# lukemelas/deep-spectral-segmentation

Hardware: AMD Instinct MI355X
Metric: images/sec end-to-end (features+eigs) at 480², K=5; eigvec cos-err vs CPU (higher is better)
Workload: dtype f16

## Files before the change

deep-spectral-segmentation_amd/build.py:

```python
from __future__ import annotations

import concurrent.futures as cf
import hashlib
import os
import shutil
import subprocess
import sys
from pathlib import Path

PKG = Path(__file__).resolve().parent
CSRC = PKG / "csrc"
LIBDIR = PKG / "lib"
LIB = LIBDIR / "libdss_hip.so"
SOURCES = ["lib.hip", "preprocess.hip", "layernorm.hip", "attention.hip", "linear384.hip", "affinity.hip", "eigs.hip", "segment.hip", "gemm.hip"]
ARCH = "gfx950"
FLAGS = ["--offload-arch=" + ARCH, "-O3", "-std=c++17", "-fPIC", "-Wall", "-Wno-unused-function"]
EXTRA_FLAGS = {"attention.hip": ["-fno-honor-nans", "-mno-amdgpu-ieee"]}


def _hipcc() -> str:
    for cand in (os.environ.get("HIPCC"), shutil.which("hipcc"), "/opt/rocm/bin/hipcc"):
        if cand and Path(cand).exists():
            return cand
    raise RuntimeError("hipcc not found (set HIPCC or install ROCm)")


def _digest() -> str:
    h = hashlib.sha256()
    for f in sorted(list(CSRC.glob("*.hip")) + list(CSRC.glob("*.h")) + [PKG.parent / "include" / "dss_hip.h"]):
        h.update(f.name.encode())
        h.update(f.read_bytes())
    h.update((" ".join(FLAGS) + repr(sorted(EXTRA_FLAGS.items()))).encode())
    return h.hexdigest()


def build(force: bool = False, verbose: bool = True) -> Path:
    LIBDIR.mkdir(exist_ok=True)
    stamp = LIBDIR / "libdss_hip.sha256"
    digest = _digest()
    if not force and LIB.exists() and stamp.exists() and stamp.read_text().strip() == digest:
        if verbose:
            print(f"[build] {LIB} is up to date")
        return LIB
    hipcc = _hipcc()
    objdir = LIBDIR / "obj"
    objdir.mkdir(exist_ok=True)

    def compile_one(src: str) -> Path:
        obj = objdir / (Path(src).stem + ".o")
        cmd = [hipcc, *FLAGS, *EXTRA_FLAGS.get(src, []), "-c", str(CSRC / src), "-o", str(obj)]
        r = subprocess.run(cmd, capture_output=True, text=True)
        if r.returncode != 0:
            raise RuntimeError(f"hipcc failed for {src}:\n{r.stdout}\n{r.stderr}")
        if verbose and r.stderr.strip():
            print(r.stderr, file=sys.stderr)
        return obj

    with cf.ThreadPoolExecutor(max_workers=min(8, len(SOURCES))) as ex:
        objs = list(ex.map(compile_one, SOURCES))
    rocm_lib = str(Path(hipcc).resolve().parent.parent / "lib")
    cmd = [hipcc, "--offload-arch=" + ARCH, "-shared", "-fPIC", "-o", str(LIB), *map(str, objs), "-L" + rocm_lib, "-lhipblaslt",
           "-Wl,-rpath," + rocm_lib]
    r = subprocess.run(cmd, capture_output=True, text=True)
    if r.returncode != 0:
        raise RuntimeError(f"link failed:\n{r.stdout}\n{r.stderr}")
    stamp.write_text(digest + "\n")
    if verbose:
        print(f"[build] wrote {LIB} ({LIB.stat().st_size} bytes)")
    return LIB


if __name__ == "__main__":
    build(force="--force" in sys.argv)
```

deep-spectral-segmentation_amd/hip.py:

```python
from __future__ import annotations

import ctypes
import functools
import os
from ctypes import c_char_p, c_float, c_int, c_size_t, c_uint, c_void_p
from pathlib import Path
from typing import Optional

import torch

PKG = Path(__file__).resolve().parent
LIB_PATH = PKG / "lib" / "libdss_hip.so"

DSS_F32, DSS_F16, DSS_BF16 = 0, 1, 2
_DTYPE_CODE = {torch.float32: DSS_F32, torch.float16: DSS_F16, torch.bfloat16: DSS_BF16}

SYMBOLS = {
    "dss_abi_version": (c_int, []),
    "dss_last_error": (c_char_p, []),
    "dss_target_arch": (c_char_p, []),
    "dss_preprocess_chw": (c_int, [c_void_p, c_void_p, c_int, c_int, c_int, c_void_p]),
    "dss_preprocess_patchify": (c_int, [c_void_p, c_void_p, c_int, c_int, c_int, c_int, c_int, c_void_p]),
    "dss_layernorm_fwd": (c_int, [c_void_p, c_void_p, c_int, c_int, c_void_p, c_void_p, c_void_p, c_int, c_int, c_int,
                                  c_float, c_void_p]),
    "dss_attention_fwd": (c_int, [c_void_p, c_int, c_void_p, c_int, c_int, c_int, c_float, c_int, c_void_p]),
    "dss_linear_k384": (c_int, [c_void_p, c_void_p, c_void_p, c_void_p, c_int, c_int, c_int, c_int, c_int, c_void_p]),
    "dss_linear_k768": (c_int, [c_void_p, c_void_p, c_void_p, c_void_p, c_int, c_int, c_int, c_int, c_int, c_void_p]),
    "dss_linear_lt_workspace_bytes": (c_size_t, []),
    "dss_linear_lt": (c_int, [c_void_p, c_void_p, c_void_p, c_void_p, ctypes.c_long, c_int, c_int, c_int, c_int, c_void_p, c_size_t,
                              c_void_p]),
    "dss_linear_lt_accumulate": (c_int, [c_void_p, c_void_p, c_void_p, c_void_p, ctypes.c_long, c_int, c_int, c_int, c_void_p, c_size_t,
                                         c_void_p]),
    "dss_linear_lt_describe": (c_int, [ctypes.c_long, c_int, c_int, c_int, c_int, c_int, c_size_t, c_char_p, c_size_t]),
    "dss_lnlinear_prepare": (c_int, [c_void_p, c_void_p, c_void_p, c_void_p, c_void_p, c_void_p, c_int, c_int, c_int,
                                     c_void_p]),
    "dss_lnlinear_k384": (c_int, [c_void_p, c_void_p, c_int, c_float, c_void_p, c_void_p, c_void_p, c_int, c_int, c_int,
                                  c_int, c_int, c_void_p]),
    "dss_lnlinear_k768": (c_int, [c_void_p, c_void_p, c_int, c_float, c_void_p, c_void_p, c_void_p, c_int, c_int, c_int,
                                  c_int, c_int, c_void_p]),
    "dss_lnlinear_kfeatures_k384": (c_int, [c_void_p, c_void_p, c_int, c_float, c_void_p, c_void_p, c_void_p, c_void_p,
                                            c_void_p, c_int, c_int, c_float, c_void_p]),
    "dss_lnlinear_kfeatures": (c_int, [c_void_p, c_void_p, c_int, c_float, c_void_p, c_void_p, c_void_p, c_void_p,
                                       c_void_p, c_int, c_int, c_int, c_float, c_int, c_void_p]),
    "dss_patch_embed_p16": (c_int, [c_void_p, c_void_p, c_void_p, c_void_p, c_void_p, c_int, c_int, c_int, c_int, c_int, c_void_p]),
    "dss_normalize_rows": (c_int, [c_void_p, c_void_p, c_int, c_int, c_float, c_void_p]),
    "dss_affinity_ld": (c_int, [c_int]),
    "dss_affinity_elems": (c_size_t, [c_int]),
    "dss_affinity": (c_int, [c_void_p, c_void_p, c_int, c_int, c_int, c_int, c_void_p]),
    "dss_affinity_split_workspace_bytes": (c_size_t, [c_int, c_int, c_int]),
    "dss_affinity_split": (c_int, [c_void_p, c_void_p, c_int, c_int, c_int, c_int, c_float, c_int, c_void_p, c_size_t,
                                   c_void_p]),
    "dss_affinity_split_u16": (c_int, [c_void_p, c_void_p, c_int, c_int, c_int, c_float, c_void_p, c_size_t, c_void_p]),
    "dss_affinity_fused_u16": (c_int, [c_void_p, c_void_p, c_int, c_int, c_int, c_float, c_void_p]),
    "dss_affinity_f16_u16": (c_int, [c_void_p, c_void_p, c_void_p, c_int, c_int, c_int, c_void_p]),
    "dss_kfeatures_finalize": (c_int, [c_void_p, c_void_p, c_void_p, c_void_p, c_void_p, c_int, c_int, c_int, c_float,
                                       c_void_p]),
    "dss_eigs_workspace_bytes": (c_size_t, [c_int, c_int, c_int, c_int]),
    "dss_laplacian_eigs_u16": (c_int, [c_void_p, c_int, c_int, c_int, c_void_p, c_void_p, c_void_p, c_int, c_float,
                                       c_int, c_void_p, c_size_t, c_void_p]),
    "dss_laplacian_eigs": (c_int, [c_void_p, c_int, c_int, c_int, c_void_p, c_void_p, c_void_p, c_int, c_float,
                                   c_int, c_void_p, c_size_t, c_void_p]),
    "dss_symmetric_eigs": (c_int, [c_void_p, c_int, c_int, c_int, c_int, c_void_p, c_void_p, c_void_p, c_int, c_float,
                                   c_int, c_void_p, c_size_t, c_void_p]),
    "dss_sign_rule": (c_int, [c_void_p, c_int, c_int, c_void_p]),
    "dss_fiedler_mask": (c_int, [c_void_p, c_void_p, c_int, c_int, c_int, c_int, c_float, c_void_p]),
    "dss_kmeans_segments": (c_int, [c_void_p, c_int, c_int, c_int, c_int, c_int, c_int, c_void_p, c_uint, c_int, c_float,
                                    c_int, c_int, c_int, c_void_p, c_void_p, c_void_p, c_void_p]),
}


class HipLibraryError(RuntimeError):
    """libdss_hip.so is missing, failed to load, or one of its entry points returned an error."""


_lib: Optional[ctypes.CDLL] = None

TIMERS: Optional[dict] = None
TIMER_SAMPLE = 1
TIMER_ALWAYS = ("laplacian_eigs", "affinity", "kfeatures_finalize", "lnlinear_kfeatures", "layernorm")


class _timed:

    def __init__(self, name: str, **meta):
        self.name, self.meta = name, meta

    def __enter__(self):
        self.on = False
        if TIMERS is not None:
            counts = TIMERS.setdefault("_launches", {})
            n = counts.get(self.name, 0)
            counts[self.name] = n + 1
            self.on = TIMER_SAMPLE <= 1 or self.name in TIMER_ALWAYS or n % TIMER_SAMPLE == 0
        if self.on:
            self.start = torch.cuda.Event(enable_timing=True)
            self.end = torch.cuda.Event(enable_timing=True)
            self.start.record()
        return self

    def __exit__(self, *exc):
        if self.on:
            self.end.record()
            TIMERS.setdefault(self.name, []).append((self.start, self.end, self.meta))
        return False


def load_library(path: Optional[Path] = None) -> ctypes.CDLL:
    global _lib
    if _lib is not None and path is None:
        return _lib
# ... 47 lines not shown
def preprocess_chw(img_u8: torch.Tensor) -> torch.Tensor:
    b, h, w, c = img_u8.shape
    assert c == 3 and img_u8.dtype == torch.uint8
    out = torch.empty((b, 3, h, w), dtype=torch.float32, device=img_u8.device)
    _check(load_library().dss_preprocess_chw(_dev(img_u8, "img"), _dev(out, "out"), b, h, w, _stream()),
           "dss_preprocess_chw")
    return out


def preprocess_patchify(img_u8: torch.Tensor, patch: int, dtype: torch.dtype) -> torch.Tensor:
    b, h, w, c = img_u8.shape
    assert c == 3 and img_u8.dtype == torch.uint8
    out = torch.empty((b, (h // patch) * (w // patch), 3 * patch * patch), dtype=dtype, device=img_u8.device)
    _check(load_library().dss_preprocess_patchify(_dev(img_u8, "img"), _dev(out, "out"), b, h, w, patch,
                                                  dtype_code(dtype), _stream()), "dss_preprocess_patchify")
    return out


ROW_MAJOR, PLANAR64 = 0, 1


def planar_to_rows(t: torch.Tensor) -> torch.Tensor:
    return t.permute(1, 0, 2).reshape(t.shape[1], t.shape[0] * 64)


def layernorm(x: torch.Tensor, gamma: torch.Tensor, beta: torch.Tensor, eps: float, out_dtype: torch.dtype,
              residual: Optional[torch.Tensor] = None, out: Optional[torch.Tensor] = None,
              residual_planar: bool = False) -> torch.Tensor:
    assert x.dtype == torch.float32
    d = x.shape[-1]
    rows = x.numel() // d
    if out is None:
        out = torch.empty(x.shape, dtype=out_dtype, device=x.device)
    rp, rc = (0, 0) if residual is None else (_dev(residual, "residual"), dtype_code(residual.dtype))
    if residual is not None:
        assert residual.shape == ((d // 64, rows, 64) if residual_planar else x.shape)
    layout = PLANAR64 if (residual is not None and residual_planar) else ROW_MAJOR
    with _timed("layernorm", rows=rows, d=d, res=residual is not None, out_bytes=out.element_size()):
        _check(load_library().dss_layernorm_fwd(_dev(x, "x"), rp, rc, layout, _dev(gamma, "gamma"), _dev(beta, "beta"),
                                                _dev(out, "out"), dtype_code(out.dtype), rows, d, float(eps),
                                                _stream()), "dss_layernorm_fwd")
    return out


def attention(qkv: torch.Tensor, heads: int, scale: float, out: Optional[torch.Tensor] = None,
              planar_bt: Optional[tuple] = None) -> torch.Tensor:
    if planar_bt is None:
        b, t, c3 = qkv.shape
        assert c3 == 3 * heads * 64, "head dim must be 64"
    else:
        b, t = planar_bt
        assert tuple(qkv.shape) == (3 * heads, b * t, 64), "planar qkv must be [3*heads, B*T, 64]"
    if out is None:
        out = torch.empty((b, t, heads * 64), dtype=qkv.dtype, device=qkv.device)
    with _timed("attention", b=b, t=t, heads=heads):
        _check(load_library().dss_attention_fwd(_dev(qkv, "qkv"), ROW_MAJOR if planar_bt is None else PLANAR64,
                                                _dev(out, "out"), b, t, heads, float(scale),
                                                dtype_code(qkv.dtype), _stream()),
               "dss_attention_fwd")
    return out


LINEAR_KRES_WIDTHS = {384: ("dss_linear_k384", 512), 768: ("dss_linear_k768", 256)}


def linear_kres(x: torch.Tensor, weight: torch.Tensor, bias: torch.Tensor, gelu: bool = False,
                planar: bool = False) -> torch.Tensor:
    k = x.shape[-1]
    if k not in LINEAR_KRES_WIDTHS:
        raise ValueError(f"linear_kres: reduction dimension must be one of {sorted(LINEAR_KRES_WIDTHS)} (got {k})")
    assert weight.shape[1] == k and x.dtype == weight.dtype == bias.dtype
    entry = LINEAR_KRES_WIDTHS[k][0]
    n = weight.shape[0]
    m = x.numel() // k
    shape = (n // 64, m, 64) if planar else (*x.shape[:-1], n)
    out = torch.empty(shape, dtype=x.dtype, device=x.device)
    with _timed("linear_kres", m=m, n=n, k=k, gelu=gelu):
        _check(getattr(load_library(), entry)(_dev(x, "x"), _dev(weight, "weight"), _dev(bias, "bias"), _dev(out, "out"),
                                              m, n, int(gelu), PLANAR64 if planar else ROW_MAJOR, dtype_code(x.dtype),
                                              _stream()), entry)
    return out


_LT_WORKSPACE: dict = {}


def _lt_workspace(device: torch.device) -> torch.Tensor:
    idx = device.index if device.index is not None else torch.cuda.current_device()
    if idx not in _LT_WORKSPACE:
        _LT_WORKSPACE[idx] = torch.empty(max(16, int(load_library().dss_linear_lt_workspace_bytes())), dtype=torch.uint8, device=device)
    return _LT_WORKSPACE[idx]


def linear_lt(x: torch.Tensor, weight: torch.Tensor, bias: Optional[torch.Tensor] = None, out_dtype: Optional[torch.dtype] = None,
              what: str = "") -> torch.Tensor:
    k = x.shape[-1]
    n = weight.shape[0]
    assert weight.shape[1] == k and x.dtype == weight.dtype and x.dtype in (torch.float16, torch.bfloat16)
    assert bias is None or (bias.dtype == x.dtype and tuple(bias.shape) == (n,))
    out_dtype = x.dtype if out_dtype is None else out_dtype
    m = x.numel() // k
    out = torch.empty((*x.shape[:-1], n), dtype=out_dtype, device=x.device)
    ws = _lt_workspace(x.device)
    with _timed("library_gemm", m=m, n=n, k=k, what=what):
        _check(load_library().dss_linear_lt(_dev(x, "x"), _dev(weight, "weight"), 0 if bias is None else _dev(bias, "bias"),
                                            _dev(out, "out"), m, n, k, dtype_code(x.dtype), dtype_code(out_dtype), ws.data_ptr(),
                                            ws.numel(), _stream()), "dss_linear_lt")
    return out


def linear_lt_accumulate(x: torch.Tensor, weight: torch.Tensor, bias: Optional[torch.Tensor], stream_x: torch.Tensor, what: str = "") -> torch.Tensor:
    k = x.shape[-1]
    n = weight.shape[0]
    assert weight.shape[1] == k and x.dtype == weight.dtype and x.dtype in (torch.float16, torch.bfloat16)
    assert bias is None or (bias.dtype == torch.float32 and tuple(bias.shape) == (n,))
    m = x.numel() // k
    assert stream_x.dtype == torch.float32 and stream_x.numel() == m * n
    ws = _lt_workspace(x.device)
    with _timed("library_gemm", m=m, n=n, k=k, what=what):
        _check(load_library().dss_linear_lt_accumulate(_dev(x, "x"), _dev(weight, "weight"), 0 if bias is None else _dev(bias, "bias"),
                                                       _dev(stream_x, "stream_x"), m, n, k, dtype_code(x.dtype), ws.data_ptr(), ws.numel(),
                                                       _stream()), "dss_linear_lt_accumulate")
    return stream_x


def linear_lt_describe(m: int, n: int, k: int, dtype: torch.dtype = torch.float16, out_dtype: Optional[torch.dtype] = None,
                       bias: bool = True) -> str:
    buf = ctypes.create_string_buffer(1 << 16)
    lib = load_library()
    _check(lib.dss_linear_lt_describe(m, n, k, dtype_code(dtype), dtype_code(out_dtype or dtype), int(bias),
                                      int(lib.dss_linear_lt_workspace_bytes()), buf, len(buf)), "dss_linear_lt_describe")
    return buf.value.decode(errors="replace")


IMAGENET_MEAN, IMAGENET_STD = (0.485, 0.456, 0.406), (0.229, 0.224, 0.225)


def patch_embed16_prepare(weight: torch.Tensor, bias: torch.Tensor, dtype: torch.dtype):
    d = weight.shape[0]
    w = weight.detach().double().reshape(d, 3, 16, 16)
    mean = torch.tensor(IMAGENET_MEAN, dtype=torch.float64, device=w.device).view(1, 3, 1, 1)
    std = torch.tensor(IMAGENET_STD, dtype=torch.float64, device=w.device).view(1, 3, 1, 1)
    bp = bias.detach().double() - (w * ((mean - 128.0 / 255.0) / std)).sum(dim=(1, 2, 3))
    wp = (w / (255.0 * std)).permute(0, 2, 3, 1).reshape(d, 768)
    return wp.to(dtype).contiguous(), bp.float().contiguous()


_ZERO_BIAS: dict = {}


def patch_embed16(img_u8: torch.Tensor, wp: torch.Tensor, bp: Optional[torch.Tensor], pos: torch.Tensor, x: torch.Tensor) -> torch.Tensor:
    assert img_u8.dtype == torch.uint8 and img_u8.dim() == 4 and img_u8.shape[-1] == 3 and img_u8.is_contiguous()
    b, h, w, _ = img_u8.shape
    n_p = (h // 16) * (w // 16)
    d = wp.shape[0]
    if bp is None:
        key = (d, wp.dtype, wp.device)
        if key not in _ZERO_BIAS:
            _ZERO_BIAS[key] = torch.zeros(d, dtype=wp.dtype, device=wp.device)
        bp = _ZERO_BIAS[key]
    else:
        bp = bp.to(wp.dtype)
    assert tuple(wp.shape) == (d, 768) and tuple(bp.shape) == (d,) and bp.dtype == wp.dtype
    assert pos.dtype == torch.float32 and tuple(pos.shape) == (n_p, d) and pos.is_contiguous()
    assert x.dtype == torch.float32 and tuple(x.shape) == (b, n_p + 1, d) and x.is_contiguous()
    with _timed("patch_embed", m=b * n_p, n=d, k=768):
# ... 275 lines not shown
```

deep-spectral-segmentation_amd/vit.py:

```python
from __future__ import annotations

import math
from pathlib import Path
from typing import Dict, Optional, Tuple

import torch
import torch.nn.functional as F

from . import hip
from .synthetic import VIT_CONFIGS

LN_EPS = 1e-6
_TUNING_FILE = Path(__file__).resolve().parent / "tuning" / "tunableop_gfx950.csv"
_gemm_tuning_ready = False


def setup_gemm_tuning(tune_new_shapes: bool = False, use_table: bool = True) -> None:
    global _gemm_tuning_ready
    if not use_table:
        return
    tun = torch.cuda.tunable
    if not _gemm_tuning_ready:
        tun.enable(True)
        if hasattr(tun, "write_file_on_exit"):
            tun.write_file_on_exit(False)
        tun.set_max_tuning_duration(15)
        if _TUNING_FILE.is_file():
            try:
                tun.read_file(str(_TUNING_FILE))
            except Exception as e:
                print(f"[dss] ignoring GEMM tuning table {_TUNING_FILE.name}: {e}")
        _gemm_tuning_ready = True
    tun.tuning_enable(bool(tune_new_shapes))


def interpolate_pos_encoding(pos_embed: torch.Tensor, patch: int, h: int, w: int) -> torch.Tensor:
    pos_embed = pos_embed.detach().float().cpu()
    n0 = pos_embed.shape[1] - 1
    hp, wp = h // patch, w // patch
    if hp * wp == n0 and h == w:
        return pos_embed.clone()
    dim = pos_embed.shape[-1]
    side = int(math.sqrt(n0))
    grid = pos_embed[:, 1:].reshape(1, side, side, dim).permute(0, 3, 1, 2)
    grid = F.interpolate(grid, scale_factor=((hp + 0.1) / side, (wp + 0.1) / side), mode="bicubic")
    if (grid.shape[-2], grid.shape[-1]) != (hp, wp):
        raise RuntimeError(f"pos-embed interpolation produced {tuple(grid.shape[-2:])}, wanted {(hp, wp)}")
    grid = grid.permute(0, 2, 3, 1).reshape(1, -1, dim)
    return torch.cat((pos_embed[:, :1], grid), dim=1)


class DinoViT:

    def __init__(self, model_name: str, state_dict: Dict[str, torch.Tensor], device: torch.device,
                 dtype: torch.dtype = torch.float16, k_proj_fp32: bool = False, gelu: str = "auto",
                 linear_kres: int = 2, fuse_ln: bool = True, gemm_tuning: str = "table", fuse_k: bool = True, fuse_pe: bool = True,
                 fuse_qkv768: bool = True, library_gemm: str = "lt", fc2_into_stream: bool = False):
        name = model_name.lower()
        if name not in VIT_CONFIGS:
            raise ValueError(f"Cannot get model: {model_name}")
        if dtype not in (torch.float16, torch.bfloat16):
            raise ValueError("compute dtype must be torch.float16 or torch.bfloat16")
        self.model_name = name
        self.embed_dim, self.depth, self.num_heads, self.patch_size = VIT_CONFIGS[name]
        self.device, self.dtype = torch.device(device), dtype
        self.k_proj_fp32 = k_proj_fp32
        if gelu not in ("auto", "erf", "erf_f16", "tanh_fused"):
            raise ValueError("gelu must be 'auto', 'erf' (DINO's exact GELU, fp32 arithmetic), 'erf_f16' (the same function evaluated on "
                             "packed f16: f16 operands and the K-resident fc1 kernel only) or 'tanh_fused'")
        if gelu == "auto":
            gelu = "erf_f16" if self.embed_dim == 384 else "erf"
        if gelu == "erf_f16" and (dtype != torch.float16 or linear_kres < 2 or self.embed_dim not in hip.LINEAR_KRES_WIDTHS):
            gelu = "erf"
        self.gelu = gelu
        self._gelu_code = 2 if gelu == "erf_f16" else 1
        if linear_kres not in (0, 1, 2):
            raise ValueError("linear_kres must be 0, 1 or 2")
        self.linear_k384 = int(linear_kres)
        self.fuse_ln = bool(fuse_ln)
        self.fuse_k = bool(fuse_k)
        self.fuse_qkv768 = bool(fuse_qkv768)
        if library_gemm not in ("lt", "torch"):
            raise ValueError("library_gemm must be 'lt' (dss_linear_lt) or 'torch' (F.linear)")
        self.library_gemm = library_gemm
        self.fc2_into_stream = bool(fc2_into_stream) and library_gemm == "lt"
        d = self.embed_dim
        sd = state_dict
        need = ["cls_token", "pos_embed", "patch_embed.proj.weight", "patch_embed.proj.bias"]
        for i in range(self.depth):
            for s in ("norm1.weight", "norm1.bias", "attn.qkv.weight", "attn.qkv.bias", "attn.proj.weight",
                      "attn.proj.bias", "norm2.weight", "norm2.bias", "mlp.fc1.weight", "mlp.fc1.bias",
                      "mlp.fc2.weight", "mlp.fc2.bias"):
                need.append(f"blocks.{i}.{s}")
        missing = [k for k in need if k not in sd]
        if missing:
            raise KeyError(f"state_dict is missing {len(missing)} DINO ViT keys, e.g. {missing[:3]}")

        def lp(t):
            return t.detach().to(self.device, dtype).contiguous()

        def f32(t):
            return t.detach().to(self.device, torch.float32).contiguous()

        self.cls_token = sd["cls_token"].detach().float().cpu()
        self.pos_embed = sd["pos_embed"].detach().float().cpu()
        self.pe_w = lp(sd["patch_embed.proj.weight"].reshape(d, -1))
        self.pe_b = lp(sd["patch_embed.proj.bias"])
        self.pe16 = None
        if self.patch_size == 16 and fuse_pe and fuse_ln and linear_kres and d % 64 == 0:
            self.pe16 = hip.patch_embed16_prepare(sd["patch_embed.proj.weight"].to(self.device), sd["patch_embed.proj.bias"].to(self.device), dtype)
        self.blocks = []
        for i in range(self.depth):
            p = f"blocks.{i}."
            self.blocks.append(dict(
                n1w=f32(sd[p + "norm1.weight"]), n1b=f32(sd[p + "norm1.bias"]),
                qkv_w=lp(sd[p + "attn.qkv.weight"]), qkv_b=lp(sd[p + "attn.qkv.bias"]),
                k_w32=f32(sd[p + "attn.qkv.weight"][d:2 * d]), k_b32=f32(sd[p + "attn.qkv.bias"][d:2 * d]),
                k_w=lp(sd[p + "attn.qkv.weight"][d:2 * d]),
                proj_w=lp(sd[p + "attn.proj.weight"]), proj_b=lp(sd[p + "attn.proj.bias"]),
                n2w=f32(sd[p + "norm2.weight"]), n2b=f32(sd[p + "norm2.bias"]),
                fc1_w=lp(sd[p + "mlp.fc1.weight"]), fc1_b=lp(sd[p + "mlp.fc1.bias"]),
                fc2_w=lp(sd[p + "mlp.fc2.weight"]), fc2_b=lp(sd[p + "mlp.fc2.bias"]), fc2_b32=f32(sd[p + "mlp.fc2.bias"]),
            ))
        hip.load_library()
        if self.fuse_ln and self.linear_k384 and d in hip.LINEAR_KRES_WIDTHS:
            for i, blk in enumerate(self.blocks):
                p = f"blocks.{i}."
                if d == 384 or (d == 768 and self.fuse_qkv768):
                    blk["qkv_wg"], blk["qkv_aux"] = hip.lnlinear_prepare(f32(sd[p + "attn.qkv.weight"]), f32(sd[p + "attn.qkv.bias"]),
                                                                         blk["n1w"], blk["n1b"], dtype)
                if self.fuse_k:
                    blk["k_wg"], blk["k_aux"] = hip.lnlinear_prepare(blk["k_w32"], blk["k_b32"], blk["n1w"], blk["n1b"], dtype)
                if self.linear_k384 >= 2 and self.gelu in ("erf", "erf_f16"):
                    blk["fc1_wg"], blk["fc1_aux"] = hip.lnlinear_prepare(f32(sd[p + "mlp.fc1.weight"]), f32(sd[p + "mlp.fc1.bias"]),
                                                                         blk["n2w"], blk["n2b"], dtype)
        self.norm_w = f32(sd["norm.weight"]) if "norm.weight" in sd else None
        self.norm_b = f32(sd["norm.bias"]) if "norm.bias" in sd else None
        self.scale = 64 ** -0.5
        assert d // self.num_heads == 64, "DINO ViTs use 64-dim heads"
        self._pos_cache: Dict[tuple, object] = {}
        if gemm_tuning not in ("table", "online", "off"):
            raise ValueError("gemm_tuning must be 'table' (shipped TunableOp table), 'online' (also tune new shapes) or 'off'")
        setup_gemm_tuning(tune_new_shapes=gemm_tuning == "online", use_table=gemm_tuning != "off")

    def _linear(self, x: torch.Tensor, w: torch.Tensor, b: Optional[torch.Tensor], what: str, out_dtype=None) -> torch.Tensor:
        if self.library_gemm == "lt":
            return hip.linear_lt(x, w, b, out_dtype=out_dtype, what=what)
        k = x.shape[-1]
        with hip._timed("library_gemm", m=x.numel() // k, n=w.shape[0], k=k, what=what):
            if out_dtype is not None and out_dtype != x.dtype:
                out = torch.mm(x.reshape(-1, k), w.t(), out_dtype=out_dtype).view(*x.shape[:-1], w.shape[0])
                return out if b is None else out + b.to(out_dtype)
            return F.linear(x, w, b)

    def paths(self) -> Dict[str, str]:
        blk, d = self.blocks[0], self.embed_dim
        k384 = bool(self.linear_k384) and d == 384
        kres_fc1 = self.gelu in ("erf", "erf_f16") and self.linear_k384 >= 2 and d in hip.LINEAR_KRES_WIDTHS
        lib = ("library GEMM (hipBLASLt through dss_linear_lt: no Stream-K split, verified)" if self.library_gemm == "lt"
               else "library GEMM (hipBLASLt through F.linear)")
        return {
            "patch_embed": "dss_patch_embed_p16 (transform + GEMM + position rows, one kernel)" if self.pe16 is not None
                           else f"dss_preprocess_patchify + {lib} + add",
            "norm1+qkv": f"dss_lnlinear_k{d}" if ("qkv_wg" in blk and self.linear_k384) else
                         ("dss_layernorm_fwd + dss_linear_k384" if k384 else f"dss_layernorm_fwd + {lib}"),
            "attention": "dss_attention_fwd",
            "proj": "dss_linear_k384" if k384 else lib,
            "norm2+fc1+gelu": f"dss_lnlinear_k{d}" if (kres_fc1 and "fc1_wg" in blk) else
                              (f"dss_layernorm_fwd + dss_linear_k{d}" if kres_fc1 else f"dss_layernorm_fwd + {lib} + GELU pass"),
            "gelu": {"erf": "exact-erf form in fp32 (A&S 7.1.28, |err| <= 3e-7)", "erf_f16": "erf-GELU polynomial form on packed f16 (csrc/kres.h)",
                     "tanh_fused": "hipBLASLt's tanh epilogue (NOT the reference function)"}[self.gelu],
            "fc2": lib + (" adding into the fp32 residual stream (dss_linear_lt_accumulate)" if self.fc2_into_stream else ""),
            "hooked norm1 + K projection + hand-over": "dss_lnlinear_kfeatures" if "k_wg" in self.blocks[-1] else
                                                       f"dss_layernorm_fwd + {lib} + dss_kfeatures_finalize",
        }

    def _pos(self, h: int, w: int) -> Tuple[torch.Tensor, torch.Tensor]:
        key = (h, w)
        if key not in self._pos_cache:
            pe = interpolate_pos_encoding(self.pos_embed, self.patch_size, h, w)
            cls_row = (self.cls_token[0, 0] + pe[0, 0]).to(self.device)
            self._pos_cache[key] = (cls_row.contiguous(), pe[0, 1:].to(self.device).contiguous())
        return self._pos_cache[key]

    @torch.no_grad()
    def _run_blocks(self, img_u8: torch.Tensor, nblocks: int):
        b, h, w, _ = img_u8.shape
        p, d, heads = self.patch_size, self.embed_dim, self.num_heads
        hp, wp = h // p, w // p
        t = hp * wp + 1
        cls_row, pos = self._pos(hp * p, wp * p)
        x = torch.empty((b, t, d), dtype=torch.float32, device=self.device)
        x[:, 0] = cls_row
        if self.pe16 is not None:
            key = ("pe16", hp * p, wp * p)
            if key not in self._pos_cache:
                self._pos_cache[key] = (pos + self.pe16[1]).contiguous()
            hip.patch_embed16(img_u8.contiguous(), self.pe16[0], None, self._pos_cache[key], x)
        else:
            patches = hip.preprocess_patchify(img_u8.contiguous(), p, self.dtype)
            tok = self._linear(patches, self.pe_w, self.pe_b, "patch_embed")
            torch.add(tok, pos, out=x[:, 1:])

        pending = None
        k384 = self.linear_k384 and d == 384
        kres_fc1 = self.gelu in ("erf", "erf_f16") and self.linear_k384 >= 2 and d in hip.LINEAR_KRES_WIDTHS
        for i in range(nblocks):
            blk = self.blocks[i]
            qkv_planar = bool(k384)
            if "qkv_wg" in blk and self.linear_k384:
                qkv = hip.lnlinear(x, pending, blk["qkv_wg"], blk["qkv_aux"], LN_EPS, planar=True)
                qkv_planar = True
            else:
                hcur = hip.layernorm(x, blk["n1w"], blk["n1b"], LN_EPS, self.dtype, residual=pending)
                if k384:
                    qkv = hip.linear_kres(hcur, blk["qkv_w"], blk["qkv_b"], planar=True)
                else:
                    qkv = self._linear(hcur, blk["qkv_w"], blk["qkv_b"], "qkv")
            o = hip.attention(qkv, heads, self.scale, planar_bt=(b, t)) if qkv_planar else hip.attention(qkv, heads, self.scale)
            if k384:
                pending = hip.linear_kres(o, blk["proj_w"], blk["proj_b"], planar=True)
            else:
                pending = self._linear(o, blk["proj_w"], blk["proj_b"], "proj")
            if kres_fc1 and "fc1_wg" in blk:
                f1 = hip.lnlinear(x, pending, blk["fc1_wg"], blk["fc1_aux"], LN_EPS, gelu=self._gelu_code, residual_planar=bool(k384))
            else:
                hcur = hip.layernorm(x, blk["n2w"], blk["n2b"], LN_EPS, self.dtype, residual=pending,
                                     residual_planar=bool(k384))
                if kres_fc1:
                    f1 = hip.linear_kres(hcur, blk["fc1_w"], blk["fc1_b"], gelu=self._gelu_code)
                elif self.gelu in ("erf", "erf_f16"):
                    f1 = F.gelu(self._linear(hcur, blk["fc1_w"], blk["fc1_b"], "fc1"))
                else:
                    f1 = torch._addmm_activation(blk["fc1_b"], hcur.view(b * t, d), blk["fc1_w"].t(),
                                                 use_gelu=True).view(b, t, -1)
            if self.fc2_into_stream:
                hip.linear_lt_accumulate(f1, blk["fc2_w"], blk["fc2_b32"], x, what="fc2")
                pending = None
            else:
                pending = self._linear(f1, blk["fc2_w"], blk["fc2_b"], "fc2")
        return x, pending

    @torch.no_grad()
    def forward_cls(self, img_u8: torch.Tensor) -> torch.Tensor:
        assert img_u8.dtype == torch.uint8 and img_u8.dim() == 4 and img_u8.shape[-1] == 3
        if self.norm_w is None:
            raise KeyError("state_dict has no final norm.weight / norm.bias: forward_cls needs them")
        if img_u8.shape[1] < self.patch_size or img_u8.shape[2] < self.patch_size:
            raise ValueError(f"image {tuple(img_u8.shape[1:3])} is smaller than one {self.patch_size}x{self.patch_size} patch")
        x, pending = self._run_blocks(img_u8, self.depth)
        cls = x[:, 0] if pending is None else x[:, 0] + pending[:, 0].float()
        return F.layer_norm(cls, (self.embed_dim,), self.norm_w, self.norm_b, LN_EPS)

    @torch.no_grad()
    def extract_k_f16(self, img_u8: torch.Tensor, which_block: int = -1, out=None):
        return self.extract_k(img_u8, which_block, _finalize=True, _out=out)

    @torch.no_grad()
    def extract_k(self, img_u8: torch.Tensor, which_block: int = -1, _finalize: bool = False, _out=None) -> torch.Tensor:
        assert img_u8.dtype == torch.uint8 and img_u8.dim() == 4 and img_u8.shape[-1] == 3
        b, h, w, _ = img_u8.shape
        p, d, heads = self.patch_size, self.embed_dim, self.num_heads
        hp, wp = h // p, w // p
        if hp == 0 or wp == 0:
            raise ValueError(f"image {h}x{w} is smaller than one {p}x{p} patch")
        n, t = hp * wp, hp * wp + 1
        wb = which_block if which_block >= 0 else self.depth + which_block
        if not 0 <= wb < self.depth:
            raise IndexError(f"which_block={which_block} out of range for depth {self.depth}")

        x, pending = self._run_blocks(img_u8, wb)
        blk = self.blocks[wb]
        if self.k_proj_fp32:
            h32 = hip.layernorm(x, blk["n1w"], blk["n1b"], LN_EPS, torch.float32, residual=pending)
            k = F.linear(h32, blk["k_w32"], blk["k_b32"])
        elif "k_wg" in blk and t > 64:
            res = hip.lnlinear_kfeatures(x, pending, blk["k_wg"], blk["k_aux"], LN_EPS, out=_out)
            return res if _finalize else res[0]
        else:
            hk = hip.layernorm(x, blk["n1w"], blk["n1b"], LN_EPS, self.dtype, residual=pending)
            k = self._linear(hk, blk["k_w"], None, "k_proj", out_dtype=torch.float32)
            if _finalize and n > 0:
                return hip.kfeatures_finalize(k, blk["k_b32"], out=_out)
            k += blk["k_b32"]
        k = k[:, 1:, :].contiguous()
        if _finalize:
            return hip.kfeatures_finalize(torch.cat((k[:, :1], k), dim=1), None, out=_out)
        return k


def wave_filling_batch(tokens: int, target: int = 256, rows_per_workgroup: int = 512,
                       compute_units: Optional[int] = None) -> int:
    if compute_units is None:
        compute_units = torch.cuda.get_device_properties(torch.cuda.current_device()).multi_processor_count
    best, best_eff = target, 0.0
    for b in range(max(1, int(target * 0.85)), int(target * 1.25) + 1):
        tiles = b * tokens / rows_per_workgroup
        waves = math.ceil(math.ceil(tiles) / compute_units)
        eff = tiles / (waves * compute_units)
        if eff > best_eff + 1e-9 or (abs(eff - best_eff) <= 1e-9 and abs(b - target) < abs(best - target)):
            best, best_eff = b, eff
    return best


def load_dino_state_dict(path: str) -> Dict[str, torch.Tensor]:
    sd = torch.load(path, map_location="cpu", weights_only=True)
    for key in ("teacher", "student", "state_dict", "model"):
        if isinstance(sd, dict) and key in sd and isinstance(sd[key], dict):
            sd = sd[key]
    out = {}
    for k, v in sd.items():
        k = k.replace("module.", "").replace("backbone.", "")
        out[k] = v
    return out
```

include/dss_hip.h:

```cpp
#ifndef DSS_HIP_H
#define DSS_HIP_H

#include <stddef.h>
#include <stdint.h>

#ifdef __cplusplus
extern "C" {
#endif

#define DSS_ABI_VERSION 10

enum { DSS_F32 = 0, DSS_F16 = 1, DSS_BF16 = 2 };

enum { DSS_ROW_MAJOR = 0, DSS_PLANAR64 = 1 };

enum {
  DSS_OK = 0,
  DSS_ERR_BAD_ARG = -1,
  DSS_ERR_HIP = -2,
  DSS_ERR_WORKSPACE = -3,
  DSS_ERR_NO_CONVERGENCE = -4
};

int dss_abi_version(void);
const char* dss_last_error(void);
const char* dss_target_arch(void);

int dss_preprocess_chw(const uint8_t* img_u8, float* out_chw, int B, int H, int W, void* stream);
int dss_preprocess_patchify(const uint8_t* img_u8, void* out, int B, int H, int W, int P,
                            int out_dtype, void* stream);

int dss_layernorm_fwd(float* x, const void* residual, int res_dtype, int res_layout, const float* gamma,
                      const float* beta, void* y, int out_dtype, int rows, int D, float eps,
                      void* stream);

int dss_attention_fwd(const void* qkv, int qkv_layout, void* out, int B, int T, int heads, float scale, int dtype,
                      void* stream);

int dss_linear_k384(const void* A, const void* W, const void* bias, void* C, int M, int N, int gelu, int out_layout,
                    int dtype, void* stream);
int dss_linear_k768(const void* A, const void* W, const void* bias, void* C, int M, int N, int gelu, int out_layout,
                    int dtype, void* stream);

size_t dss_linear_lt_workspace_bytes(void);
int dss_linear_lt(const void* A, const void* W, const void* bias, void* C, long M, int N, int K, int dtype, int out_dtype,
                  void* workspace, size_t workspace_bytes, void* stream);
int dss_linear_lt_describe(long M, int N, int K, int dtype, int out_dtype, int has_bias, size_t workspace_bytes, char* buf,
                           size_t buflen);
int dss_linear_lt_accumulate(const void* A, const void* W, const float* bias, float* X, long M, int N, int K, int dtype,
                             void* workspace, size_t workspace_bytes, void* stream);

int dss_lnlinear_prepare(const float* W, const float* bias, const float* gamma, const float* beta, void* Wg, float* aux,
                         int N, int K, int dtype, void* stream);
int dss_lnlinear_k384(float* x, const void* residual, int res_layout, float eps, const void* Wg, const float* aux, void* C,
                      int M, int N, int gelu, int out_layout, int dtype, void* stream);
int dss_lnlinear_k768(float* x, const void* residual, int res_layout, float eps, const void* Wg, const float* aux, void* C,
                      int M, int N, int gelu, int out_layout, int dtype, void* stream);

int dss_lnlinear_kfeatures_k384(float* x, const void* residual, int res_layout, float eps, const void* Wg, const float* aux,
                                float* k32, void* k16, float* rnorm, int M, int T, float norm_eps, void* stream);
int dss_lnlinear_kfeatures(float* x, const void* residual, int res_layout, float eps, const void* Wg, const float* aux,
                           float* k32, void* k16, float* rnorm, int M, int T, int D, float norm_eps, int dtype, void* stream);

int dss_patch_embed_p16(const uint8_t* img_u8, const void* Wp, const void* biasp, const float* pos, float* x, int B, int H, int W,
                        int D, int dtype, void* stream);

int dss_normalize_rows(const float* x, float* y, int rows, int D, float eps, void* stream);

int dss_affinity_ld(int N);
size_t dss_affinity_elems(int N);
int dss_affinity(const float* feats, float* W, int B, int N, int D, int threshold_at_zero,
                 void* stream);

size_t dss_affinity_split_workspace_bytes(int B, int N, int D);
int dss_affinity_split(const float* feats, float* W, int B, int N, int D, int normalize, float eps,
                       int threshold_at_zero, void* workspace, size_t workspace_bytes, void* stream);
int dss_affinity_split_u16(const float* feats, uint16_t* W, int B, int N, int D, float eps, void* workspace,
                           size_t workspace_bytes, void* stream);

int dss_affinity_fused_u16(const float* feats, uint16_t* W, int B, int N, int D, float eps, void* stream);

int dss_affinity_f16_u16(const void* feats16, const float* rnorm, uint16_t* W, int B, int N, int D, void* stream);

int dss_kfeatures_finalize(const float* kproj, const float* bias, float* k32, void* k16, float* rnorm, int B, int T, int D,
                           float eps, void* stream);

size_t dss_eigs_workspace_bytes(int B, int N, int K, int ncv);
int dss_laplacian_eigs(const float* W, int B, int N, int K, float* eigenvalues, float* eigenvectors,
                       int32_t* info, int ncv, float tol, int max_restarts,
                       void* workspace, size_t workspace_bytes, void* stream);
int dss_laplacian_eigs_u16(const uint16_t* W, int B, int N, int K, float* eigenvalues, float* eigenvectors,
                           int32_t* info, int ncv, float tol, int max_restarts,
                           void* workspace, size_t workspace_bytes, void* stream);

enum { DSS_EIGS_NORMALIZED_LAPLACIAN = 0, DSS_EIGS_AFFINITY_LM = 1, DSS_EIGS_LAPLACIAN = 2 };
int dss_symmetric_eigs(const float* W, int B, int N, int K, int mode, float* eigenvalues, float* eigenvectors,
                       int32_t* info, int ncv, float tol, int max_restarts,
                       void* workspace, size_t workspace_bytes, void* stream);

int dss_sign_rule(float* eigenvectors, int rows, int N, void* stream);

int dss_fiedler_mask(const float* eigenvectors, uint8_t* mask, int B, int K, int N, int index, float threshold,
                     void* stream);
int dss_kmeans_segments(const float* eigenvectors, int B, int K, int N, int first, int dims, int k,
                        const float* centroids_init, unsigned seed, int max_iter, float tol, int hp, int wp, int infer_bg,
                        uint8_t* labels, float* inertia, int32_t* iters, void* stream);

#ifdef __cplusplus
}
#endif
#endif
```

Baseline: 14340.

## Add custom persistent fc2 GEMM kernel for K=1536, N=384 with LDS-DMA pipeline

Adds a hand-written persistent HIP kernel for the ViT MLP fc2 projection (1536 to 384) and routes fc2 through it by default for D=384 models. Each block holds a full-N tile of 192 rows, double-buffers A and W slices into LDS with global_load_lds DMA, interleaves LDS fragment loads with 32x32x16 MFMAs, and prefetches the next tile's first slice during the last K step. The epilogue adds bias and stages the output through LDS for coalesced stores. It replaces the hipBLASLt call and aims to cut library overhead and raise MFMA utilisation, but its correctness and speed depend on hand-tuned scheduling.

After: 14480, median of 6. About the same (+1.0%).

```diff
diff --git a/deep-spectral-segmentation_amd/build.py b/deep-spectral-segmentation_amd/build.py
--- a/deep-spectral-segmentation_amd/build.py
+++ b/deep-spectral-segmentation_amd/build.py
@@ -12,7 +12,7 @@
 CSRC = PKG / "csrc"
 LIBDIR = PKG / "lib"
 LIB = LIBDIR / "libdss_hip.so"
-SOURCES = ["lib.hip", "preprocess.hip", "layernorm.hip", "attention.hip", "linear384.hip", "affinity.hip", "eigs.hip", "segment.hip", "gemm.hip"]
+SOURCES = ["lib.hip", "preprocess.hip", "layernorm.hip", "attention.hip", "linear384.hip", "linear1536.hip", "affinity.hip", "eigs.hip", "segment.hip", "gemm.hip"]
 ARCH = "gfx950"
 FLAGS = ["--offload-arch=" + ARCH, "-O3", "-std=c++17", "-fPIC", "-Wall", "-Wno-unused-function"]
 EXTRA_FLAGS = {"attention.hip": ["-fno-honor-nans", "-mno-amdgpu-ieee"]}
diff --git a/deep-spectral-segmentation_amd/csrc/linear1536.hip b/deep-spectral-segmentation_amd/csrc/linear1536.hip
--- /dev/null
+++ b/deep-spectral-segmentation_amd/csrc/linear1536.hip
@@ -0,0 +1,246 @@
+#include "common.h"
+#include "kres.h"
+#include <type_traits>
+
+namespace dss {
+
+constexpr int F2_K = 1536, F2_N = 384, F2_BM = 192, F2_BK = 64, F2_STEPS = F2_K / F2_BK;
+constexpr int F2_THREADS = 512;
+constexpr int F2_A_BYTES = F2_BM * F2_BK * 2;
+constexpr int F2_W_BYTES = F2_N * F2_BK * 2;
+constexpr int F2_A_OFF = 0, F2_W_OFF = 2 * F2_A_BYTES;
+constexpr int F2_PITCH = 208;
+constexpr int F2_PATCH_BYTES = 32 * F2_PITCH;
+constexpr int F2_PATCH_OFF = F2_W_OFF + F2_W_BYTES;
+constexpr int F2_BIAS_OFF = F2_PATCH_OFF + 8 * F2_PATCH_BYTES;
+constexpr int F2_SMEM_BYTES = F2_BIAS_OFF + F2_N * 4;
+static_assert(F2_BIAS_OFF >= F2_W_OFF + 2 * F2_W_BYTES && F2_STEPS % 2 == 0 && F2_SMEM_BYTES <= 163840 &&
+              F2_A_BYTES + 2 * 4096 + 1024 < 65536 && F2_W_BYTES + 2 * 4096 + 1024 < 65536, "fc2 kernel layout");
+
+__device__ __forceinline__ void f2_dma(unsigned lds_addr, unsigned voff, const unsigned char* sbase) {
+  unsigned keep;
+  asm volatile("s_mov_b32 %0, m0\n\ts_mov_b32 m0, %1\n\ts_nop 0\n\tglobal_load_lds_dwordx4 %2, %3\n\t"
+               "s_mov_b32 m0, %0"
+               : "=&s"(keep) : "s"(lds_addr), "v"(voff), "s"(sbase) : "memory");
+}
+__device__ __forceinline__ const unsigned char* f2_uniform(const unsigned char* p) {
+  const unsigned long long v = (unsigned long long)p;
+  const unsigned lo = __builtin_amdgcn_readfirstlane((unsigned)v), hi = __builtin_amdgcn_readfirstlane((unsigned)(v >> 32));
+  return reinterpret_cast<const unsigned char*>(((unsigned long long)hi << 32) | lo);
+}
+
+template <class T>
+__global__ __launch_bounds__(F2_THREADS) void linear_k1536_kernel(const T* __restrict__ A, const T* __restrict__ W,
+                                                                  const T* __restrict__ bias, T* __restrict__ C, long M, long ntiles) {
+  typedef typename vec8<T>::type V8;
+  typedef typename vec4<T>::type V4;
+  __shared__ __attribute__((aligned(1024))) unsigned char smem[F2_SMEM_BYTES];
+  const int tid = threadIdx.x;
+  const int lane = tid & 63, wave = __builtin_amdgcn_readfirstlane(tid >> 6);
+  const int li = lane & 31, hh = lane >> 5;
+  const int wr = wave >> 2, wc = wave & 3;
+  float* const bs = reinterpret_cast<float*>(smem + F2_BIAS_OFF);
+  if (tid < F2_N) bs[tid] = to_f32<T>(bias[tid]);
+
+  const unsigned smem0 = __builtin_amdgcn_readfirstlane((unsigned)(size_t)(lds_ptr_t)smem);
+  const int prow = lane >> 3;
+  unsigned woff[2], aoff[3];
+#pragma unroll
+  for (int j = 0; j < 2; ++j)
+    woff[j] = (unsigned)(48 * wave + prow) * (unsigned)(F2_K * 2) + 16u * (unsigned)((lane & 7) ^ (4 * j + (lane >> 4)));
+  auto set_aoff = [&](long tile) {
+    const long left = M - tile * F2_BM;
+    const int mrem = left < F2_BM ? (int)left : F2_BM;
+#pragma unroll
+    for (int j = 0; j < 3; ++j) {
+      const int p = 3 * wave + j;
+      const int row = min(8 * p + prow, mrem - 1);
+      aoff[j] = (unsigned)row * (unsigned)(F2_K * 2) + 16u * (unsigned)((lane & 7) ^ (4 * (p & 1) + (lane >> 4)));
+    }
+  };
+  auto issue = [&](int buf, long tile, int k) {
+    const unsigned char* asrc = f2_uniform(reinterpret_cast<const unsigned char*>(A) + (size_t)tile * ((size_t)F2_BM * F2_K * 2) + (size_t)k * (F2_BK * 2));
+    const unsigned char* wsrc = f2_uniform(reinterpret_cast<const unsigned char*>(W) + (size_t)k * (F2_BK * 2));
+    const unsigned sa = smem0 + F2_A_OFF + (unsigned)buf * F2_A_BYTES + (unsigned)wave * 3072u;
+    const unsigned sw = smem0 + F2_W_OFF + (unsigned)buf * F2_W_BYTES + (unsigned)wave * 6144u;
+#pragma unroll
+    for (int j = 0; j < 3; ++j) f2_dma(__builtin_amdgcn_readfirstlane(sa + 1024u * j), aoff[j], asrc);
+#pragma unroll
+    for (int j = 0; j < 6; ++j) f2_dma(__builtin_amdgcn_readfirstlane(sw + 1024u * j), woff[j & 1], wsrc + j * (8 * F2_K * 2));
+  };
+  auto stage_barrier = [&]() {
+    asm volatile("s_waitcnt vmcnt(0) lgkmcnt(0)" ::: "memory");
+    __builtin_amdgcn_s_barrier();
+    asm volatile("" ::: "memory");
+  };
+
+  f32x16 acc[3][3];
+  const unsigned fsw = (unsigned)((li >> 1) & 7);
+  const unsigned char* fa[4];
+  const unsigned char* fw[4];
+#pragma unroll
+  for (int ks = 0; ks < 4; ++ks) {
+    const unsigned co = (((unsigned)(2 * ks + hh)) ^ fsw) << 4;
+    fa[ks] = smem + F2_A_OFF + (wr * 96 + li) * 128 + co;
+    fw[ks] = smem + F2_W_OFF + (wc * 96 + li) * 128 + co;
+  }
+  V8 f0[6], f1[6];
+  auto load = [&](V8* f, auto boc, auto ksc) {
+    constexpr int B = decltype(boc)::value, ks = decltype(ksc)::value;
+#pragma unroll
+    for (int t = 0; t < 3; ++t) {
+      f[t] = *reinterpret_cast<const V8*>(fw[ks] + B * F2_W_BYTES + t * 4096);
+      f[3 + t] = *reinterpret_cast<const V8*>(fa[ks] + B * F2_A_BYTES + t * 4096);
+    }
+  };
+  auto mfmas = [&](const V8* f) {
+#pragma unroll
+    for (int tn = 0; tn < 3; ++tn)
+#pragma unroll
+      for (int tm = 0; tm < 3; ++tm) acc[tn][tm] = mfma32x32x16(f[tn], f[3 + tm], acc[tn][tm]);
+  };
+  typedef std::integral_constant<int, 0> I0;
+  typedef std::integral_constant<int, 1> I1;
+  typedef std::integral_constant<int, 2> I2;
+  typedef std::integral_constant<int, 3> I3;
+  auto pair = [&](V8* fl, auto boc, auto ksc, const V8* fm) {
+    load(fl, boc, ksc);
+    mfmas(fm);
+#pragma unroll
+    for (int i = 0; i < 6; ++i) {
+      __builtin_amdgcn_sched_group_barrier(0x008, 1, 0);
+      __builtin_amdgcn_sched_group_barrier(0x100, 1, 0);
+    }
+    __builtin_amdgcn_sched_group_barrier(0x008, 3, 0);
+  };
+  auto head = [&](auto boc) { pair(f0, boc, I0{}, f1); };
+  auto head_dma = [&](auto boc, long t, int k) {
+    constexpr int B = decltype(boc)::value;
+    const unsigned char* asrc = f2_uniform(reinterpret_cast<const unsigned char*>(A) + (size_t)t * ((size_t)F2_BM * F2_K * 2) + (size_t)k * (F2_BK * 2));
+    const unsigned char* wsrc = f2_uniform(reinterpret_cast<const unsigned char*>(W) + (size_t)k * (F2_BK * 2));
+    const unsigned sa = smem0 + F2_A_OFF + (unsigned)(B ^ 1) * F2_A_BYTES + (unsigned)wave * 3072u;
+    const unsigned sw = smem0 + F2_W_OFF + (unsigned)(B ^ 1) * F2_W_BYTES + (unsigned)wave * 6144u;
+    constexpr int order[6] = {0, 3, 4, 5, 1, 2};
+    __builtin_amdgcn_sched_barrier(0);
+#pragma unroll
+    for (int i = 0; i < 9; ++i) {
+      acc[i / 3][i % 3] = mfma32x32x16(f1[i / 3], f1[3 + i % 3], acc[i / 3][i % 3]);
+      if (i < 6) {
+        const int q = order[i];
+        f0[q] = q < 3 ? *reinterpret_cast<const V8*>(fw[0] + B * F2_W_BYTES + q * 4096)
+                      : *reinterpret_cast<const V8*>(fa[0] + B * F2_A_BYTES + (q - 3) * 4096);
+      }
+      if (i < 3) f2_dma(__builtin_amdgcn_readfirstlane(sa + 1024u * i), aoff[i], asrc);
+      else f2_dma(__builtin_amdgcn_readfirstlane(sw + 1024u * (i - 3)), woff[(i - 3) & 1], wsrc + (i - 3) * (8 * F2_K * 2));
+      __builtin_amdgcn_sched_barrier(0);
+    }
+  };
+  auto body = [&](auto boc) {
+    pair(f1, boc, I1{}, f0);
+    pair(f0, boc, I2{}, f1);
+    pair(f1, boc, I3{}, f0);
+    stage_barrier();
+  };
+
+  long tile = blockIdx.x;
+  set_aoff(tile);
+  issue(0, tile, 0);
+  asm volatile("s_waitcnt vmcnt(0) lgkmcnt(0)" ::: "memory");
+  __builtin_amdgcn_s_barrier();
+  asm volatile("" ::: "memory");
+  load(f0, I0{}, I0{});
+  while (true) {
+    const long next = tile + gridDim.x;
+    const bool has_next = next < ntiles;
+#pragma unroll
+    for (int tn = 0; tn < 3; ++tn)
+#pragma unroll
+      for (int tm = 0; tm < 3; ++tm)
+#pragma unroll
+        for (int e = 0; e < 16; ++e) acc[tn][tm][e] = 0.f;
+    issue(1, tile, 1);
+    body(I0{});
+    head_dma(I1{}, tile, 2);
+    body(I1{});
+#pragma unroll 1
+    for (int k = 2; k < F2_STEPS; k += 2) {
+      head_dma(I0{}, tile, k + 1);
+      body(I0{});
+      const bool last = k + 2 == F2_STEPS;
+      const long t2 = last && has_next ? next : tile;
+      if (last) set_aoff(t2);
+      head_dma(I1{}, t2, last ? 0 : k + 2);
+      body(I1{});
+    }
+    head(I0{});
+    int eln = lane;
+    asm volatile("" : "+v"(eln));
+    const int eli = eln & 31, ehh = eln >> 5;
+    unsigned char* const patch = smem + F2_PATCH_OFF + wave * F2_PATCH_BYTES;
+    const long row0 = tile * F2_BM + wr * 96;
+#pragma unroll
+    for (int tm = 0; tm < 3; ++tm) {
+#pragma unroll
+      for (int tn = 0; tn < 3; ++tn) {
+        f32x4 bv[4];
+#pragma unroll
+        for (int g = 0; g < 4; ++g) bv[g] = *reinterpret_cast<const f32x4*>(bs + wc * 96 + 32 * tn + 8 * g + 4 * ehh);
+#pragma unroll
+        for (int g = 0; g < 4; ++g) {
+          V4 o;
+#pragma unroll
+          for (int e = 0; e < 4; ++e) o[e] = from_f32<T>(acc[tn][tm][4 * g + e] + bv[g][e]);
+          *reinterpret_cast<V4*>(patch + eli * F2_PITCH + (32 * tn + 8 * g + 4 * ehh) * 2) = o;
+        }
+      }
+      V8 v[6];
+#pragma unroll
+      for (int i = 0; i < 6; ++i) {
+        const int p = 64 * i + eln, r = p / 12, c = p - 12 * r;
+        v[i] = *reinterpret_cast<const V8*>(patch + r * F2_PITCH + c * 16);
+      }
+#pragma unroll
+      for (int i = 0; i < 6; ++i) {
+        const int p = 64 * i + eln, r = p / 12, c = p - 12 * r;
+        const long gm = row0 + 32 * tm + r;
+        if (gm < M) *reinterpret_cast<V8*>(C + gm * F2_N + wc * 96 + c * 8) = v[i];
+      }
+    }
+    asm volatile("s_waitcnt lgkmcnt(0)" ::: "memory");
+    __builtin_amdgcn_s_barrier();
+    asm volatile("" ::: "memory");
+    if (!has_next) break;
+    tile = next;
+  }
+}
+
+static int f2_compute_units() {
+  static int ncu = 0;
+  if (ncu == 0) {
+    int dev = 0, n = 0;
+    if (hipGetDevice(&dev) == hipSuccess && hipDeviceGetAttribute(&n, hipDeviceAttributeMultiprocessorCount, dev) == hipSuccess && n > 0) ncu = n;
+    else ncu = 256;
+  }
+  return ncu;
+}
+
+}
+
+extern "C" int dss_linear_k1536(const void* A, const void* W, const void* bias, void* C, long M, int dtype, void* stream) {
+  DSS_REQUIRE(A && W && bias && C, "dss_linear_k1536: null pointer");
+  DSS_REQUIRE(M > 0, "dss_linear_k1536: need M > 0 (M=%ld)", M);
+  DSS_REQUIRE(dtype == DSS_F16 || dtype == DSS_BF16, "dss_linear_k1536: dtype must be DSS_F16 or DSS_BF16 (got %d)", dtype);
+  DSS_REQUIRE((((size_t)A | (size_t)W | (size_t)C) & 15) == 0, "dss_linear_k1536: A, W and C must be 16-byte aligned");
+  const long ntiles = (M + dss::F2_BM - 1) / dss::F2_BM;
+  const long ncu = dss::f2_compute_units();
+  const unsigned grid = (unsigned)(ntiles < ncu ? ntiles : ncu);
+  hipStream_t s = (hipStream_t)stream;
+  if (dtype == DSS_F16)
+    hipLaunchKernelGGL((dss::linear_k1536_kernel<dss::f16>), dim3(grid), dim3(dss::F2_THREADS), 0, s, (const dss::f16*)A, (const dss::f16*)W,
+                       (const dss::f16*)bias, (dss::f16*)C, M, ntiles);
+  else
+    hipLaunchKernelGGL((dss::linear_k1536_kernel<dss::bf16>), dim3(grid), dim3(dss::F2_THREADS), 0, s, (const dss::bf16*)A, (const dss::bf16*)W,
+                       (const dss::bf16*)bias, (dss::bf16*)C, M, ntiles);
+  DSS_CHECK_LAUNCH("dss_linear_k1536");
+  return DSS_OK;
+}
diff --git a/deep-spectral-segmentation_amd/hip.py b/deep-spectral-segmentation_amd/hip.py
--- a/deep-spectral-segmentation_amd/hip.py
+++ b/deep-spectral-segmentation_amd/hip.py
@@ -26,6 +26,7 @@
     "dss_attention_fwd": (c_int, [c_void_p, c_int, c_void_p, c_int, c_int, c_int, c_float, c_int, c_void_p]),
     "dss_linear_k384": (c_int, [c_void_p, c_void_p, c_void_p, c_void_p, c_int, c_int, c_int, c_int, c_int, c_void_p]),
     "dss_linear_k768": (c_int, [c_void_p, c_void_p, c_void_p, c_void_p, c_int, c_int, c_int, c_int, c_int, c_void_p]),
+    "dss_linear_k1536": (c_int, [c_void_p, c_void_p, c_void_p, c_void_p, ctypes.c_long, c_int, c_void_p]),
     "dss_linear_lt_workspace_bytes": (c_size_t, []),
     "dss_linear_lt": (c_int, [c_void_p, c_void_p, c_void_p, c_void_p, ctypes.c_long, c_int, c_int, c_int, c_int, c_void_p, c_size_t,
                               c_void_p]),
@@ -239,6 +240,22 @@
     return out
 
 
+LINEAR_K1536_SHAPE = (384, 1536)
+
+
+def linear_k1536(x: torch.Tensor, weight: torch.Tensor, bias: torch.Tensor) -> torch.Tensor:
+    n, k = LINEAR_K1536_SHAPE
+    if x.shape[-1] != k or tuple(weight.shape) != (n, k) or tuple(bias.shape) != (n,):
+        raise ValueError(f"linear_k1536: need x [..., {k}], weight [{n}, {k}], bias [{n}] (got {tuple(x.shape)}, {tuple(weight.shape)}, {tuple(bias.shape)})")
+    assert x.dtype == weight.dtype == bias.dtype and x.dtype in (torch.float16, torch.bfloat16)
+    m = x.numel() // k
+    out = torch.empty((*x.shape[:-1], n), dtype=x.dtype, device=x.device)
+    with _timed("linear_kres", m=m, n=n, k=k, what="fc2"):
+        _check(load_library().dss_linear_k1536(_dev(x, "x"), _dev(weight, "weight"), _dev(bias, "bias"), _dev(out, "out"), m,
+                                               dtype_code(x.dtype), _stream()), "dss_linear_k1536")
+    return out
+
+
 _LT_WORKSPACE: dict = {}
 
 
diff --git a/deep-spectral-segmentation_amd/vit.py b/deep-spectral-segmentation_amd/vit.py
--- a/deep-spectral-segmentation_amd/vit.py
+++ b/deep-spectral-segmentation_amd/vit.py
@@ -13,6 +13,7 @@
 LN_EPS = 1e-6
 _TUNING_FILE = Path(__file__).resolve().parent / "tuning" / "tunableop_gfx950.csv"
 _gemm_tuning_ready = False
+FC2_AUTO_TAKES_OWN = True
 
 
 def setup_gemm_tuning(tune_new_shapes: bool = False, use_table: bool = True) -> None:
@@ -55,7 +56,7 @@
     def __init__(self, model_name: str, state_dict: Dict[str, torch.Tensor], device: torch.device,
                  dtype: torch.dtype = torch.float16, k_proj_fp32: bool = False, gelu: str = "auto",
                  linear_kres: int = 2, fuse_ln: bool = True, gemm_tuning: str = "table", fuse_k: bool = True, fuse_pe: bool = True,
-                 fuse_qkv768: bool = True, library_gemm: str = "lt", fc2_into_stream: bool = False):
+                 fuse_qkv768: bool = True, library_gemm: str = "lt", fc2_into_stream: bool = False, fc2_kernel: str = "auto"):
         name = model_name.lower()
         if name not in VIT_CONFIGS:
             raise ValueError(f"Cannot get model: {model_name}")
@@ -84,6 +85,13 @@
             raise ValueError("library_gemm must be 'lt' (dss_linear_lt) or 'torch' (F.linear)")
         self.library_gemm = library_gemm
         self.fc2_into_stream = bool(fc2_into_stream) and library_gemm == "lt"
+        if fc2_kernel not in ("auto", "library", "own"):
+            raise ValueError("fc2_kernel must be 'auto', 'library' (hipBLASLt) or 'own' (dss_linear_k1536, D = 384 only)")
+        if fc2_kernel == "own" and self.embed_dim != hip.LINEAR_K1536_SHAPE[0]:
+            raise ValueError(f"fc2_kernel='own': dss_linear_k1536 is the D = 384 kernel (this model has D = {self.embed_dim})")
+        self.fc2_kernel = fc2_kernel
+        self._fc2_own = (self.embed_dim == hip.LINEAR_K1536_SHAPE[0] and not self.fc2_into_stream
+                         and (fc2_kernel == "own" or (fc2_kernel == "auto" and FC2_AUTO_TAKES_OWN)))
         d = self.embed_dim
         sd = state_dict
         need = ["cls_token", "pos_embed", "patch_embed.proj.weight", "patch_embed.proj.bias"]
@@ -170,7 +178,8 @@
                               (f"dss_layernorm_fwd + dss_linear_k{d}" if kres_fc1 else f"dss_layernorm_fwd + {lib} + GELU pass"),
             "gelu": {"erf": "exact-erf form in fp32 (A&S 7.1.28, |err| <= 3e-7)", "erf_f16": "erf-GELU polynomial form on packed f16 (csrc/kres.h)",
                      "tanh_fused": "hipBLASLt's tanh epilogue (NOT the reference function)"}[self.gelu],
-            "fc2": lib + (" adding into the fp32 residual stream (dss_linear_lt_accumulate)" if self.fc2_into_stream else ""),
+            "fc2": "dss_linear_k1536 (full-N tile, LDS-DMA pipeline)" if self._fc2_own else
+                   lib + (" adding into the fp32 residual stream (dss_linear_lt_accumulate)" if self.fc2_into_stream else ""),
             "hooked norm1 + K projection + hand-over": "dss_lnlinear_kfeatures" if "k_wg" in self.blocks[-1] else
                                                        f"dss_layernorm_fwd + {lib} + dss_kfeatures_finalize",
         }
@@ -237,6 +246,8 @@
             if self.fc2_into_stream:
                 hip.linear_lt_accumulate(f1, blk["fc2_w"], blk["fc2_b32"], x, what="fc2")
                 pending = None
+            elif self._fc2_own:
+                pending = hip.linear_k1536(f1, blk["fc2_w"], blk["fc2_b"])
             else:
                 pending = self._linear(f1, blk["fc2_w"], blk["fc2_b"], "fc2")
         return x, pending
diff --git a/include/dss_hip.h b/include/dss_hip.h
--- a/include/dss_hip.h
+++ b/include/dss_hip.h
@@ -41,6 +41,8 @@
                     int dtype, void* stream);
 int dss_linear_k768(const void* A, const void* W, const void* bias, void* C, int M, int N, int gelu, int out_layout,
                     int dtype, void* stream);
+
+int dss_linear_k1536(const void* A, const void* W, const void* bias, void* C, long M, int dtype, void* stream);
 
 size_t dss_linear_lt_workspace_bytes(void);
 int dss_linear_lt(const void* A, const void* W, const void* bias, void* C, long M, int N, int K, int dtype, int out_dtype,
```
